# BinomialLLC/basis_universal

Hardware: AMD Instinct MI355X
Metric: encoder Mpixels/s (ETC1S frontend hot path) (higher is better)
Workload: dtype u8/int32; 1 GPU; 4096x4096 synthetic RGBA (SURVEY 8d recipe, seed 1234), ETC1S -q128 comp_level 1, basisu_frontend init+compress with tiles resident in HBM; blocks=1048576, max_endpoint_clusters=2416, max_selector_clusters=2731, final_endpoint_clusters=2413, final_selector_clusters=2277, images_in_flight_per_gpu=1, parallelism=1 x one image per GPU (no collective)

## Files before the change

basis_universal_amd/csrc/api_context.cpp:

```cpp
#include <atomic>
#include <chrono>
#include <cstdarg>
#include <cstdlib>
#include "api_internal.h"
#include "etc1s_kernels.h"
#include "tsvq_kernels.h"
#include "tsvq_bufs.h"

static std::mutex g_init_mutex;
static bool g_initialized = false;
static int g_device_count = 0;
static std::string g_global_error;
static std::atomic<int> g_live_contexts{0};
static std::mutex g_park_lock;
static std::vector<bu_hip_context*> g_parked;

void set_error(bu_hip_context* ctx, const char* fmt, ...) {
    char buf[512];
    va_list ap; va_start(ap, fmt); vsnprintf(buf, sizeof(buf), fmt, ap); va_end(ap);
    if (ctx) ctx->error = buf; else g_global_error = buf;
}

hipError_t stream_wait(bu_hip_context* ctx, hipStream_t s) {
    if (!ctx->wait_hook) return hipStreamSynchronize(s);
// ... 347 lines not shown
        ctx->tuning = default_tuning();
        std::lock_guard<std::mutex> g(g_park_lock);
        if (g_parked.size() < park_limit()) { g_parked.push_back(ctx); return; }
    }
    context_release(ctx);
}

int bu_hip_context_device(const bu_hip_context* ctx) { return ctx ? ctx->device : -1; }
int bu_hip_set_stream(bu_hip_context* ctx, void* s) {
    if (!ctx) return 0;
    (void)stream_wait(ctx, ctx->stream);
    ctx->stage_used = 0;
    ctx->stream = s ? (hipStream_t)s : ctx->own_stream;
    return 1;
}
void* bu_hip_get_stream(bu_hip_context* ctx) { return ctx ? (void*)ctx->stream : nullptr; }
const char* bu_hip_last_error(const bu_hip_context* ctx) { return ctx ? ctx->error.c_str() : g_global_error.c_str(); }
void bu_hip_set_last_error(bu_hip_context* ctx, const char* text) { set_error(ctx, "%s", text ? text : ""); }

void bu_hip_get_tuning(const bu_hip_context* ctx, bu_hip_tuning* out, uint32_t struct_bytes) {
    if (!out || struct_bytes < 8) return;
    const bu_hip_tuning& t = ctx ? ctx->tuning : default_tuning();
    std::memcpy(out, &t, std::min<size_t>(struct_bytes, sizeof(t)));
    out->struct_bytes = (uint32_t)std::min<size_t>(struct_bytes, sizeof(t));
}

int bu_hip_set_tuning(bu_hip_context* ctx, const bu_hip_tuning* t) {
    if (!ctx) return 0;
    if (!t) { ctx->tuning = default_tuning(); return 1; }
    if (t->struct_bytes < 8 || t->struct_bytes > 4096) { set_error(ctx, "bu_hip_set_tuning: struct_bytes %u", t->struct_bytes); return 0; }
    bu_hip_tuning n = default_tuning();
    std::memcpy(&n, t, std::min<size_t>(t->struct_bytes, sizeof(n)));
    n.struct_bytes = (uint32_t)sizeof(n);
    if ((n.tsvq_wide_min && n.tsvq_wide_min < 512) || (n.tsvq_wide6_min && n.tsvq_wide6_min < 512) || n.tsvq_windows > 2 || n.tsvq_poll > 2 || n.tsvq_deep_levels > bu::TSVQ_MAX_DEEP_LEVELS) {
        set_error(ctx, "bu_hip_set_tuning: value out of range (many-workgroup thresholds are 0 or >= 512, windows / poll 0..2, deep levels 0..2)");
        return 0;
    }
    ctx->tuning = n;
    return 1;
}

int bu_hip_set_wait_hook(bu_hip_context* ctx, bu_hip_wait_fn fn, void* user) {
    if (!ctx) return 0;
    ctx->wait_hook = fn; ctx->wait_user = fn ? user : nullptr;
    return 1;
}

int bu_hip_sync(bu_hip_context* ctx) {
    if (!ctx) return 0;
    device_guard g(ctx->device);
    BU_TRY(ctx, stream_wait(ctx, ctx->stream));
    return 1;
}

void* bu_hip_malloc(bu_hip_context* ctx, size_t bytes) {
    if (!ctx) return nullptr;
    device_guard g(ctx->device);
    const size_t want = ((bytes ? bytes : 1) + 255) & ~(size_t)255;
    int best = -1;
    for (size_t i = 0; i < ctx->pool_free.size(); i++) {
        const size_t cap = ctx->pool_free[i].cap;
        if (cap >= want && cap <= want * 2 + ((size_t)1 << 20) && (best < 0 || cap < ctx->pool_free[(size_t)best].cap)) best = (int)i;
    }
    if (best >= 0) {
        const bu_hip_context::pooled b = ctx->pool_free[(size_t)best];
        ctx->pool_free.erase(ctx->pool_free.begin() + best);
        ctx->pool_free_bytes -= b.cap;
        ctx->pool_live.push_back(b);
// ... 152 lines not shown
```

basis_universal_amd/csrc/api_etc1s.cpp:

```cpp
#include <atomic>
#include <cstdlib>
#include "api_internal.h"
#include "etc1s_kernels.h"
#include "mipmap_kernels.h"
#include "unique_kernels.h"
#include "bookkeeping_kernels.h"
#include "kmeans_kernels.h"
#include "host/seam_translate.h"

namespace {
constexpr uint32_t UP_PIECE_BLOCKS = 65536;
constexpr uint32_t UP_SLOTS = 8, UP_EVENTS = 64;
unsigned upload_threads() {
    static const unsigned t = [] {
        unsigned want = 4;
        if (const char* e = std::getenv("BU_UPLOAD_THREADS")) { const int v = std::atoi(e); if (v >= 1 && v <= 16) want = (unsigned)v; }
        const unsigned hw = std::thread::hardware_concurrency();
        return hw ? std::min(want, std::max(1u, hw / 2)) : 1u;
    }();
    return t;
}
bool sort_size_ok(bu_hip_context* ctx, const char* fn, uint32_t n) {
    if (n <= (1u << 30)) return true;
    set_error(ctx, "%s: %u blocks: more than 2^30 in one call", fn, n);
// ... 236 lines not shown
int bu_hip_k_refit_endpoints_given_selectors(bu_hip_context* ctx, const void* d_px, const void* d_enc, uint32_t n_clusters, const uint32_t* h_offsets,
                                             const uint32_t* d_offsets, const uint32_t* d_indices, int perceptual, uint8_t* d_params, uint64_t* d_err,
                                             uint8_t* d_valid, uint64_t* d_cur_err) {
    return bu_hip_k_refit_endpoints_given_selectors_q(ctx, d_px, d_enc, n_clusters, h_offsets, d_offsets, d_indices, BU_ETC_QUALITY_UBER, perceptual, d_params, d_err, d_valid, d_cur_err);
}

int bu_hip_k_subblock_errors(bu_hip_context* ctx, const void* d_px, uint32_t n_blocks, const uint32_t* d_block_cluster, const uint8_t* d_cluster_params,
                             int perceptual, uint64_t* d_out) {
    if (!ctx) return 0;
    device_guard g(ctx->device);
    prof_scope ps(ctx, "subblock_errors");
    BU_TRY(ctx, bu::launch_subblock_errors(ctx->stream, d_px, n_blocks, d_block_cluster, d_cluster_params, perceptual != 0, d_out));
    return 1;
}

int bu_hip_k_backend_block_errors(bu_hip_context* ctx, const void* d_px, const void* d_etc_blocks, const uint32_t* d_block_cluster, const uint8_t* d_cluster_params,
                                  uint32_t first_block, uint32_t num_blocks_x, uint32_t num_blocks_y, uint32_t n_clusters, int perceptual, int with_neighbours,
                                  uint32_t* d_own_err, uint32_t* d_neighbour_err) {
    if (!ctx) return 0;
    if (!d_px || !d_etc_blocks || !d_block_cluster || !d_cluster_params || !d_own_err || (with_neighbours && !d_neighbour_err)) { set_error(ctx, "backend_block_errors: null argument"); return 0; }
    device_guard g(ctx->device);
    prof_scope ps(ctx, "backend_block_errors");
    BU_TRY(ctx, bu::launch_backend_block_errors(ctx->stream, d_px, d_etc_blocks, d_block_cluster, d_cluster_params, first_block, num_blocks_x, num_blocks_y, n_clusters, perceptual != 0,
                                                with_neighbours != 0, d_own_err, d_neighbour_err));
    return 1;
}

int bu_hip_k_refine_endpoint_clusterization(bu_hip_context* ctx, const void* d_px, uint32_t n_blocks, const uint32_t* d_block_cluster,
                                            const uint8_t* d_cluster_params, uint32_t n_clusters, uint32_t n_parents, const uint32_t* d_cand_offsets,
                                            const uint32_t* d_cand_indices, const uint8_t* d_block_parent, int perceptual, uint32_t* d_out_best) {
    if (!ctx) return 0;
    device_guard g(ctx->device);
    void* work = nullptr;
    if (const size_t wb = ctx->tuning.refine_unsorted ? 0 : bu::refine_workspace_bytes(n_clusters, n_parents)) { BU_TRY(ctx, ctx->refine_lists.reserve(wb)); work = ctx->refine_lists.p; }
    prof_scope ps(ctx, "refine_endpoint_clusterization");
    BU_TRY(ctx, bu::launch_refine_endpoint_clusterization(ctx->stream, d_px, n_blocks, d_block_cluster, d_cluster_params, n_clusters, n_parents,
                                                          d_cand_offsets, d_cand_indices, d_block_parent, perceptual != 0, d_out_best, work));
    return 1;
}

int bu_hip_k_extract_blocks(bu_hip_context* ctx, const void* d_rgba, uint32_t width, uint32_t height, uint32_t pitch_bytes, void* d_out) {
    if (!ctx) return 0;
    if (!d_rgba || !d_out || !width || !height || pitch_bytes < width * 4u) { set_error(ctx, "extract_blocks: bad arguments"); return 0; }
    device_guard g(ctx->device);
    prof_scope ps(ctx, "extract_blocks");
    BU_TRY(ctx, bu::launch_extract_blocks(ctx->stream, d_rgba, width, height, pitch_bytes, d_out));
    return 1;
}

int bu_hip_k_extract_slices(bu_hip_context* ctx, const bu_hip_slice_source* slices, uint32_t n, void* d_out) {
    if (!ctx) return 0;
    static const char* const fn = "extract_slices";
    bu::slice_table table;
    if (!checked(ctx, [&](bu::err_text e) { return bu::build_source_slices(table, fn, slices, n, d_out, e); })) return 0;
    device_guard g(ctx->device);
    uploaded_slices d;
    if (!upload_slice_table(ctx, table, d)) return 0;
    prof_scope ps(ctx, fn);
    BU_TRY(ctx, bu::launch_extract_slices(ctx->stream, static_cast<const bu_hip_slice_source*>(d.records), d.prefix, n, table.total, d_out));
    return 1;
}

int bu_hip_k_resample_rgba8(bu_hip_context* ctx, const void* d_src, uint32_t src_w, uint32_t src_h, void* d_dst, uint32_t dst_w, uint32_t dst_h,
                            const uint32_t* x_first, const uint16_t* x_pixel, const float* x_weight, const uint32_t* y_first, const uint16_t* y_pixel, const float* y_weight,
                            int x_after_y, int srgb, const float* srgb_to_linear, const uint8_t* linear_to_srgb, uint32_t num_comps) {
    if (!ctx) return 0;
    if (!d_src || !d_dst || !src_w || !src_h || !dst_w || !dst_h || !x_first || !x_pixel || !x_weight || !y_first || !y_pixel || !y_weight || !srgb_to_linear ||
        !linear_to_srgb || num_comps < 3 || num_comps > 4 || src_w > 16384 || src_h > 16384) { set_error(ctx, "resample_rgba8: bad arguments"); return 0; }
    device_guard g(ctx->device);
    const size_t nx = x_first[dst_w], ny = y_first[dst_h];
    for (uint32_t i = 0; i < nx; i++) if (x_pixel[i] >= src_w) { set_error(ctx, "resample_rgba8: x contributor out of range"); return 0; }
// ... 310 lines not shown
    if (!ctx || !ctx->d_pixel_blocks) { if (ctx) set_error(ctx, "no pixel blocks set"); return 0; }
    device_guard g(ctx->device);
    const uint32_t n = (uint32_t)ctx->total_blocks;
    arena &in = ctx->scratch[0], &o = ctx->scratch[1];
    BU_TRY(ctx, in.reserve((size_t)n * 4));
    BU_TRY(ctx, o.reserve((size_t)n * 8));
    BU_TRY(ctx, h2d(ctx, in.p, color5_inten, (size_t)n * 4));
    BU_TRY(ctx, bu::launch_determine_selectors(ctx->stream, ctx->d_pixel_blocks, n, static_cast<const uint8_t*>(in.p), nullptr, perceptual != 0, o.p));
    if (!fetch(ctx, out, o.p, (size_t)n * 8)) return 0;
    return 1;
}

int bu_hip_refine_endpoint_clusterization(bu_hip_context* ctx, const bu_block_info* info, uint32_t total_clusters, const bu_endpoint_cluster* clusters,
                                          const uint32_t* , uint32_t* out, int perceptual) {
    if (!ctx || !ctx->d_pixel_blocks) { if (ctx) set_error(ctx, "no pixel blocks set"); return 0; }
    device_guard g(ctx->device);
    const uint32_t n = (uint32_t)ctx->total_blocks;
    if (n && !out) { set_error(ctx, "refine: null pointer"); return 0; }
    bu::seam::refine_tables t;
    if (const char* e = bu::seam::translate_refine(info, n, total_clusters, clusters, t)) { set_error(ctx, "%s", e); return 0; }
    if (!n) return 1;
    const uint32_t n_parents = t.win.n_parents();

    arena &a_par = ctx->scratch[0], &a_cur = ctx->scratch[1], &a_off = ctx->scratch[2], &a_idx = ctx->scratch[3], &a_out = ctx->scratch[4];
    arena& a_bp = ctx->scratch[5];
    BU_TRY(ctx, a_par.reserve(total_clusters * 4ull)); BU_TRY(ctx, a_cur.reserve(n * 4ull)); BU_TRY(ctx, a_off.reserve(t.win.cand_offsets.size() * 4ull));
    BU_TRY(ctx, a_idx.reserve(t.win.cand_indices.size() * 4ull + 4)); BU_TRY(ctx, a_out.reserve(n * 4ull)); BU_TRY(ctx, a_bp.reserve(n));
    BU_TRY(ctx, h2d(ctx, a_par.p, t.params.data(), total_clusters * 4ull));
    BU_TRY(ctx, h2d(ctx, a_cur.p, t.block_cur.data(), n * 4ull));
    BU_TRY(ctx, h2d(ctx, a_off.p, t.win.cand_offsets.data(), t.win.cand_offsets.size() * 4ull));
    BU_TRY(ctx, h2d(ctx, a_idx.p, t.win.cand_indices.data(), t.win.cand_indices.size() * 4ull));
    BU_TRY(ctx, h2d(ctx, a_bp.p, t.win.block_parent.data(), n));
    void* work = nullptr;
    if (const size_t wb = ctx->tuning.refine_unsorted ? 0 : bu::refine_workspace_bytes(total_clusters, n_parents)) { BU_TRY(ctx, ctx->refine_lists.reserve(wb)); work = ctx->refine_lists.p; }
    BU_TRY(ctx, bu::launch_refine_endpoint_clusterization(ctx->stream, ctx->d_pixel_blocks, n, static_cast<const uint32_t*>(a_cur.p),
                                                          static_cast<const uint8_t*>(a_par.p), total_clusters, n_parents,
                                                          static_cast<const uint32_t*>(a_off.p), static_cast<const uint32_t*>(a_idx.p),
                                                          static_cast<const uint8_t*>(a_bp.p), perceptual != 0, static_cast<uint32_t*>(a_out.p), work));
    std::vector<uint32_t> pos(n);
    if (!fetch(ctx, pos.data(), a_out.p, n * 4ull)) return 0;
    for (uint32_t b = 0; b < n; b++) out[b] = clusters[pos[b]].m_cluster_index;
    return 1;
}

int bu_hip_find_optimal_selector_clusters_for_each_block(bu_hip_context* ctx, const bu_fosc_block* info, uint32_t total_input_selectors,
                                                         const bu_fosc_selector* selectors, const uint32_t* selector_cluster_indices, uint32_t* out, int perceptual) {
    if (!ctx || !ctx->d_pixel_blocks) { if (ctx) set_error(ctx, "no pixel blocks set"); return 0; }
    device_guard g(ctx->device);
    const uint32_t n = (uint32_t)ctx->total_blocks;
    if (n && (!out || !selector_cluster_indices)) { set_error(ctx, "fosc: null pointer"); return 0; }
    bu::seam::fosc_tables t;
    if (const char* e = bu::seam::translate_fosc(info, n, total_input_selectors, selectors, t)) { set_error(ctx, "%s", e); return 0; }
    if (!n) return 1;
    const uint32_t n_parents = t.win.n_parents();

    arena &a_sel = ctx->scratch[0], &a_enc = ctx->scratch[1], &a_off = ctx->scratch[2], &a_idx = ctx->scratch[3], &a_tmp = ctx->scratch[4], &a_bp = ctx->scratch[5];
    BU_TRY(ctx, a_sel.reserve(total_input_selectors * 8ull + 8)); BU_TRY(ctx, a_enc.reserve(n * 8ull + n * 4ull)); BU_TRY(ctx, a_off.reserve(t.win.cand_offsets.size() * 4ull));
    BU_TRY(ctx, a_idx.reserve(t.win.cand_indices.size() * 4ull + 4)); BU_TRY(ctx, a_tmp.reserve(n * 4ull)); BU_TRY(ctx, a_bp.reserve(n));
    uint32_t* d_out = reinterpret_cast<uint32_t*>(static_cast<uint8_t*>(a_enc.p) + n * 8ull);
    BU_TRY(ctx, h2d(ctx, a_sel.p, t.selector_blocks.data(), total_input_selectors * 8ull));
    BU_TRY(ctx, h2d(ctx, a_enc.p, t.encoded_blocks.data(), n * 8ull));
    BU_TRY(ctx, h2d(ctx, a_off.p, t.win.cand_offsets.data(), t.win.cand_offsets.size() * 4ull));
    BU_TRY(ctx, h2d(ctx, a_idx.p, t.win.cand_indices.data(), t.win.cand_indices.size() * 4ull));
    BU_TRY(ctx, h2d(ctx, a_bp.p, t.win.block_parent.data(), n));
    BU_TRY(ctx, bu::launch_find_optimal_selector_clusters(ctx->stream, ctx->d_pixel_blocks, a_enc.p, n, a_sel.p, total_input_selectors, n_parents,
                                                          static_cast<const uint32_t*>(a_off.p), static_cast<const uint32_t*>(a_idx.p), static_cast<const uint8_t*>(a_bp.p),
                                                          perceptual != 0, 0, static_cast<uint32_t*>(a_tmp.p), d_out, nullptr, 0));
    std::vector<uint32_t> pos(n);
    if (!fetch(ctx, pos.data(), d_out, n * 4ull)) return 0;
    for (uint32_t b = 0; b < n; b++) out[b] = selector_cluster_indices[pos[b]];
    return 1;
// ... 33 lines not shown
```

basis_universal_amd/csrc/etc1s_kernels.h:

```cpp
#pragma once
#include <hip/hip_runtime.h>
#include <stdint.h>
#include <vector>
#include "../../include/basisu_hip.h"

namespace bu {

enum { BU_Q_FAST = 0, BU_Q_MEDIUM = 1, BU_Q_SLOW = 2, BU_Q_UBER = 3 };

hipError_t upload_block_fit_tables();
hipError_t upload_cluster_fit_tables();

hipError_t launch_encode_etc1s_blocks(hipStream_t st, const void* d_pixel_blocks, uint32_t n_blocks, int quality, bool perceptual, void* d_out);
hipError_t launch_endpoint_training_vectors(hipStream_t st, const void* d_etc_blocks, uint32_t n_blocks, float* d_out6);
hipError_t launch_selector_training_vectors(hipStream_t st, const void* d_enc_blocks, uint32_t n_blocks, bool perceptual, float* d_out16, uint64_t* d_w);
hipError_t launch_generate_endpoint_codebook(hipStream_t st, const void* d_pixel_blocks, uint32_t n_clusters, const uint32_t* d_order,
                                             const uint32_t* d_offsets, const uint32_t* d_indices, int quality, bool perceptual, uint32_t step,
                                             uint8_t* d_params, uint64_t* d_err, uint8_t* d_valid);
struct cb_wide_layout { size_t states_at, chunks_at, sum_at, total, image_bytes; uint32_t n_big, n_chunks; };
cb_wide_layout codebook_wide_prepare(const uint32_t* h_cluster, const uint32_t* h_first, const uint32_t* h_subblocks, uint32_t n_big, std::vector<unsigned char>& image);
hipError_t launch_codebook_wide_means(hipStream_t st, const void* d_pixel_blocks, const uint32_t* d_indices, void* d_work, const cb_wide_layout& L, float* d_out );
hipError_t launch_codebook_wide(hipStream_t st, const void* d_pixel_blocks, const uint32_t* d_indices, void* d_work, const cb_wide_layout& L, int quality, bool perceptual, bool forced,
                                uint32_t step, const void* d_enc_blocks, uint8_t* d_params, uint64_t* d_err, uint8_t* d_valid, uint64_t* d_cur_err);
hipError_t launch_refit_endpoints_given_selectors(hipStream_t st, const void* d_pixel_blocks, const void* d_enc_blocks, uint32_t n_clusters, const uint32_t* d_order,
                                                  const uint32_t* d_offsets, const uint32_t* d_indices, int quality, bool perceptual, uint8_t* d_params, uint64_t* d_err,
                                                  uint8_t* d_valid, uint64_t* d_cur_err);
hipError_t launch_subblock_errors(hipStream_t st, const void* d_pixel_blocks, uint32_t n_blocks, const uint32_t* d_block_cluster, const uint8_t* d_cluster_params,
                                  bool perceptual, uint64_t* d_out);
hipError_t launch_backend_block_errors(hipStream_t st, const void* d_pixel_blocks, const void* d_etc_blocks, const uint32_t* d_block_cluster, const uint8_t* d_cluster_params,
                                       uint32_t first_block, uint32_t nbx, uint32_t nby, uint32_t n_clusters, bool perceptual, bool with_neighbours, uint32_t* d_own,
                                       uint32_t* d_neighbour);
hipError_t launch_refine_endpoint_clusterization(hipStream_t st, const void* d_pixel_blocks, uint32_t n_blocks, const uint32_t* d_block_cluster,
                                                 const uint8_t* d_cluster_params, uint32_t n_clusters, uint32_t n_parents, const uint32_t* d_cand_offsets,
                                                 const uint32_t* d_cand_indices, const uint8_t* d_block_parent, bool perceptual, uint32_t* d_out_best,
                                                 void* d_work );
size_t refine_workspace_bytes(uint32_t n_clusters, uint32_t n_parents);
hipError_t launch_determine_selectors(hipStream_t st, const void* d_pixel_blocks, uint32_t n_blocks, const uint8_t* d_color5_inten,
                                      const uint32_t* d_block_cluster, bool perceptual, void* d_out);
size_t create_optimized_selector_codebook_workspace_bytes(uint32_t n_clusters);
hipError_t launch_create_optimized_selector_codebook(hipStream_t st, const void* d_pixel_blocks, const void* d_enc_blocks, uint32_t n_clusters,
                                                     const uint32_t* d_offsets, const uint32_t* d_block_indices, bool perceptual,
                                                     void* d_workspace, void* d_selector_blocks);
hipError_t launch_find_optimal_selector_clusters(hipStream_t st, const void* d_pixel_blocks, void* d_enc_blocks, uint32_t n_blocks,
                                                 const void* d_selector_blocks, uint32_t n_selectors, uint32_t n_parents, const uint32_t* d_cand_offsets,
                                                 const uint32_t* d_cand_indices, const uint8_t* d_block_parent, bool perceptual, uint32_t chunk,
                                                 uint32_t* d_scratch_idx, uint32_t* d_out_idx, uint32_t* d_cand_words , size_t cand_words_capacity );

hipError_t launch_extract_blocks(hipStream_t st, const void* d_rgba, uint32_t width, uint32_t height, uint32_t pitch_bytes, void* d_out_blocks);
hipError_t launch_extract_slices(hipStream_t st, const bu_hip_slice_source* d_slices, const uint32_t* d_prefix, uint32_t n_slices, uint32_t total_tiles, void* d_out_blocks);

}
```

basis_universal_amd/csrc/etc1s_refine_kernels.hip:

```cpp
#include <hip/hip_runtime.h>
#include <stdint.h>
#include "etc1s_device.h"
#include "etc1s_kernels.h"
#include "launch_dispatch.h"

namespace bu {


template <bool PERCEPTUAL>
__global__ __launch_bounds__(256) void k_refine_endpoint_clusterization(
    const uint4* __restrict__ pixel_blocks, uint32_t n_blocks, const uint32_t* __restrict__ block_cluster,
    const uint32_t* __restrict__ cluster_params, uint32_t n_clusters, uint32_t n_parents,
    const uint32_t* __restrict__ cand_offsets, const uint32_t* __restrict__ cand_indices, const uint8_t* __restrict__ block_parent,
    uint32_t* __restrict__ out_best) {
    constexpr uint32_t RQ = 256;
    __shared__ uint2 s_q[4][2][RQ];
    __shared__ uint32_t s_qp[4][2][RQ];
    const uint32_t lane = threadIdx.x & 63u;
    const uint32_t block = (uint32_t)__builtin_amdgcn_readfirstlane((int)(blockIdx.x * 4u + (threadIdx.x >> 6)));
    if (block >= n_blocks) return;

    cvec pc[16];
    {
        const uint4* src = pixel_blocks + (size_t)block * 4;
// ... 361 lines not shown
#pragma unroll
                for (int i = 0; i < 3; i++) tot += min_err4<PERCEPTUAL>(pixel_cvec<PERCEPTUAL>(block_words[(REST_PX >> (4u * (part * 3u + (uint32_t)i))) & 15u]), bc);
                tot += (uint32_t)__shfl_xor((int)tot, 1, 64);
                tot += (uint32_t)__shfl_xor((int)tot, 2, 64);
                if (have && part == 0) {
                    tot += qp[j];
                    best_key = min(best_key, ((uint64_t)tot << 32) | e.y);
                    if ((e.y & 0xffffu) == cur) cur_err = tot;
                }
            }
            if (attempt == 0) tighten();
            __builtin_amdgcn_wave_barrier();
        }
        if (seen_cur || attempt == 1) break;
        thr = 0xFFFFFFFFu; best_key = ~0ull; cur_err = 0xFFFFFFFFu;
    }
#pragma unroll
    for (int o = 32; o >= 1; o >>= 1) {
        const uint32_t lo = (uint32_t)__shfl_xor((int)(uint32_t)best_key, o, 64);
        const uint32_t hi = (uint32_t)__shfl_xor((int)(uint32_t)(best_key >> 32), o, 64);
        best_key = min(best_key, ((uint64_t)hi << 32) | lo);
        cur_err = min(cur_err, (uint32_t)__shfl_xor((int)cur_err, o, 64));
    }
    if (lane == 0) {
        const uint32_t min_err = (uint32_t)(best_key >> 32);
        uint32_t winner;
        if (best_key == ~0ull) winner = 0;
        else if (min_err != 0 && cur_err == min_err) winner = cur;
        else winner = (uint32_t)best_key & 0xffffu;
        out_best[block] = winner;
    }
}

static size_t refine_items_bytes(uint32_t n_clusters, size_t lists) { return (lists * n_clusters * sizeof(uint2) + 255) & ~(size_t)255; }

size_t refine_workspace_bytes(uint32_t n_clusters, uint32_t n_parents) {
    if (n_clusters > 65535u) return 0;
    const size_t lists = n_parents ? n_parents : 1;
    return refine_items_bytes(n_clusters, lists) + lists * RS_SEG * sizeof(uint32_t);
}

hipError_t launch_refine_endpoint_clusterization(hipStream_t st, const void* d_pixel_blocks, uint32_t n_blocks, const uint32_t* d_block_cluster,
                                                 const uint8_t* d_cluster_params, uint32_t n_clusters, uint32_t n_parents, const uint32_t* d_cand_offsets,
                                                 const uint32_t* d_cand_indices, const uint8_t* d_block_parent, bool perceptual, uint32_t* d_out_best, void* d_work) {
    if (!n_blocks) return hipSuccess;
    const dim3 grid((n_blocks + 3) / 4), blk(256);
    const uint4* in = static_cast<const uint4*>(d_pixel_blocks);
    const uint32_t* prm = reinterpret_cast<const uint32_t*>(d_cluster_params);
    const bool sorted = d_work && refine_workspace_bytes(n_clusters, n_parents);
    with_bool(perceptual, [&](auto p) {
        constexpr bool P = decltype(p)::value;
        if (sorted) {
            const size_t lists = n_parents ? n_parents : 1;
            uint2* items = static_cast<uint2*>(d_work);
            uint32_t* seg = reinterpret_cast<uint32_t*>(static_cast<char*>(d_work) + refine_items_bytes(n_clusters, lists));
            hipLaunchKernelGGL(k_refine_sort_lists<P>, dim3((uint32_t)lists), blk, 0, st, prm, n_clusters, n_parents, d_cand_offsets, d_cand_indices, items, seg);
            hipLaunchKernelGGL(k_refine_sorted<P>, grid, blk, 0, st, in, n_blocks, d_block_cluster, prm, n_parents, items, seg, d_block_parent, d_out_best);
        } else {
            hipLaunchKernelGGL(k_refine_endpoint_clusterization<P>, grid, blk, 0, st, in, n_blocks, d_block_cluster, prm, n_clusters, n_parents, d_cand_offsets, d_cand_indices,
                               d_block_parent, d_out_best);
        }
    });
    BU_LAUNCH_CHECK();
    return hipSuccess;
}

}
```

include/basisu_hip.h:

```cpp
#ifndef BASISU_HIP_H
#define BASISU_HIP_H
#include <stddef.h>
#include <stdint.h>

#ifdef __cplusplus
extern "C" {
#endif

#if defined(__GNUC__)
#define BU_HIP_API __attribute__((visibility("default")))
#else
#define BU_HIP_API
#endif


typedef struct bu_hip_context bu_hip_context;

#pragma pack(push, 1)
typedef struct { uint8_t m_pixels[16][4]; } bu_pixel_block;
typedef struct { uint8_t m_bytes[8]; } bu_etc_block;
typedef struct { uint8_t r, g, b, a; } bu_color_rgba;
typedef struct { uint64_t m_total_pixels, m_first_pixel_index; } bu_pixel_cluster;
typedef struct { uint16_t m_first_cluster_ofs, m_num_clusters, m_cur_cluster_index; uint8_t m_cur_cluster_etc_inten; } bu_block_info;
typedef struct { bu_color_rgba m_unscaled_color; uint8_t m_etc_inten; uint16_t m_cluster_index; } bu_endpoint_cluster;
// ... 100 lines not shown
    uint32_t width, height;
    uint32_t selector;
    uint32_t reserved;
} bu_hip_mip_level_record;
BU_HIP_API int bu_hip_k_prepare_mip_levels(bu_hip_context*, const void* d_payload, size_t payload_bytes, const bu_hip_mip_level_record* records, uint32_t n,
        void* d_out, size_t out_bytes, uint32_t* d_flags);

enum { BU_ETC_QUALITY_FAST = 0, BU_ETC_QUALITY_MEDIUM = 1, BU_ETC_QUALITY_SLOW = 2, BU_ETC_QUALITY_UBER = 3 };

BU_HIP_API int bu_hip_k_encode_etc1s_blocks(bu_hip_context*, const void* d_pixel_blocks, uint32_t n_blocks, int quality, int perceptual, void* d_out_etc_blocks);
BU_HIP_API int bu_hip_k_upload_and_encode_etc1s_blocks(bu_hip_context*, void* d_pixel_blocks, const void* h_pixel_blocks, uint32_t n_blocks, int quality, int perceptual,
    void* d_out_etc_blocks);
BU_HIP_API int bu_hip_k_endpoint_training_vectors(bu_hip_context*, const void* d_etc_blocks, uint32_t n_blocks, float* d_out_vec6);
BU_HIP_API int bu_hip_k_generate_endpoint_codebook(bu_hip_context*, const void* d_pixel_blocks, uint32_t n_clusters,
    const uint32_t* h_offsets, const uint32_t* d_offsets, const uint32_t* d_indices, int quality, int perceptual, uint32_t step,
    uint8_t* d_params, uint64_t* d_err, uint8_t* d_valid);
BU_HIP_API int bu_hip_k_cluster_colour_means(bu_hip_context*, const void* d_pixel_blocks, uint32_t n_clusters, const uint32_t* h_offsets, const uint32_t* d_indices, float* h_out);
BU_HIP_API int bu_hip_k_refit_endpoints_given_selectors(bu_hip_context*, const void* d_pixel_blocks, const void* d_encoded_blocks, uint32_t n_clusters,
    const uint32_t* h_offsets, const uint32_t* d_offsets, const uint32_t* d_indices, int perceptual,
    uint8_t* d_params, uint64_t* d_err, uint8_t* d_valid, uint64_t* d_current_err);
BU_HIP_API int bu_hip_k_refit_endpoints_given_selectors_q(bu_hip_context*, const void* d_pixel_blocks, const void* d_encoded_blocks, uint32_t n_clusters,
    const uint32_t* h_offsets, const uint32_t* d_offsets, const uint32_t* d_indices, int quality, int perceptual,
    uint8_t* d_params, uint64_t* d_err, uint8_t* d_valid, uint64_t* d_current_err);
BU_HIP_API int bu_hip_k_subblock_errors(bu_hip_context*, const void* d_pixel_blocks, uint32_t n_blocks, const uint32_t* d_block_cluster,
    const uint8_t* d_cluster_params, int perceptual, uint64_t* d_out_err);
BU_HIP_API int bu_hip_k_backend_block_errors(bu_hip_context*, const void* d_pixel_blocks, const void* d_etc_blocks, const uint32_t* d_block_cluster, const uint8_t* d_cluster_params,
    uint32_t first_block, uint32_t num_blocks_x, uint32_t num_blocks_y, uint32_t n_clusters, int perceptual, int with_neighbours, uint32_t* d_own_err, uint32_t* d_neighbour_err);
BU_HIP_API int bu_hip_k_generate_endpoint_codebook_part(bu_hip_context*, const void* d_pixel_blocks, uint32_t n_clusters,
    const uint32_t* h_offsets, const uint32_t* d_offsets, const uint32_t* d_indices, int quality, int perceptual, uint32_t step,
    uint8_t* d_params, uint64_t* d_err, uint8_t* d_valid, uint32_t part, uint32_t parts);
BU_HIP_API int bu_hip_k_refine_endpoint_clusterization(bu_hip_context*, const void* d_pixel_blocks, uint32_t n_blocks,
    const uint32_t* d_block_cluster, const uint8_t* d_cluster_params, uint32_t n_clusters, uint32_t n_parents,
    const uint32_t* d_cand_offsets, const uint32_t* d_cand_indices, const uint8_t* d_block_parent, int perceptual, uint32_t* d_out_best_cluster);
BU_HIP_API int bu_hip_k_resample_rgba8(bu_hip_context*, const void* d_src, uint32_t src_w, uint32_t src_h, void* d_dst, uint32_t dst_w, uint32_t dst_h,
    const uint32_t* x_first, const uint16_t* x_pixel, const float* x_weight, const uint32_t* y_first, const uint16_t* y_pixel, const float* y_weight,
    int x_after_y, int srgb, const float* srgb_to_linear_256, const uint8_t* linear_to_srgb_8192, uint32_t num_comps);
BU_HIP_API int bu_hip_k_determine_selectors(bu_hip_context*, const void* d_pixel_blocks, uint32_t n_blocks,
    const uint8_t* d_color5_inten, const uint32_t* d_block_cluster, int perceptual, void* d_out_etc_blocks);
BU_HIP_API int bu_hip_k_selector_training_vectors(bu_hip_context*, const void* d_encoded_blocks, uint32_t n_blocks, int perceptual, float* d_out_vec16, uint64_t* d_out_weight);
BU_HIP_API int bu_hip_k_create_optimized_selector_codebook(bu_hip_context*, const void* d_pixel_blocks, const void* d_encoded_blocks,
    uint32_t n_clusters, const uint32_t* d_offsets, const uint32_t* d_block_indices, int perceptual, void* d_selector_blocks);
BU_HIP_API int bu_hip_k_find_optimal_selector_clusters(bu_hip_context*, const void* d_pixel_blocks, void* d_encoded_blocks, uint32_t n_blocks,
    const void* d_selector_blocks, uint32_t n_selectors, uint32_t n_parents, const uint32_t* d_cand_offsets, const uint32_t* d_cand_indices,
    const uint8_t* d_block_parent, int perceptual, uint32_t chunk, uint32_t* d_out_block_selector_cluster);

BU_HIP_API int bu_hip_k_encode_uastc_blocks(bu_hip_context*, const void* d_pixel_blocks, uint32_t n_blocks, uint32_t flags, void* d_out_uastc_blocks);
BU_HIP_API size_t bu_hip_uastc_workspace_bytes(uint32_t n_blocks, uint32_t flags);
BU_HIP_API size_t bu_hip_uastc_rdo_workspace_bytes(uint32_t n_blocks, uint32_t total_jobs);

typedef struct bu_uastc_rdo_params {
    float m_lambda;
    float m_max_allowed_rms_increase_ratio;
    float m_skip_block_rms_thresh;
    float m_max_smooth_block_std_dev;
    float m_smooth_block_max_error_scale;
    uint32_t m_lz_dict_size;
    uint32_t m_lz_literal_cost;
    uint32_t m_endpoint_refinement;
} bu_uastc_rdo_params;
BU_HIP_API void bu_hip_uastc_rdo_default_params(bu_uastc_rdo_params* out);
BU_HIP_API int bu_hip_k_uastc_rdo(bu_hip_context*, void* d_uastc_blocks, const void* d_pixel_blocks, uint32_t n_blocks, const bu_uastc_rdo_params* params,
                                  uint32_t flags, uint32_t total_jobs, uint32_t out_stats[4]);
BU_HIP_API int bu_hip_k_uastc_rdo_slices(bu_hip_context*, void* d_uastc_blocks, const void* d_pixel_blocks, const uint32_t* slice_blocks, uint32_t n_slices,
                                         const bu_uastc_rdo_params* params, uint32_t flags, uint32_t total_jobs, uint32_t* out_stats);
BU_HIP_API size_t bu_hip_uastc_rdo_slices_workspace_bytes(const uint32_t* slice_blocks, uint32_t n_slices, uint32_t total_jobs);
BU_HIP_API int bu_hip_uastc_rdo(bu_hip_context*, bu_uastc_block* blocks, const bu_uastc_rdo_params* params, uint32_t flags, uint32_t total_jobs,
// ... 213 lines not shown
```

Before: 1240 Mpixels/s.

## Bucket blocks by parent and table for lane-per-block refine with candidate queues

Adds a new default refine path for perceptual mode. Blocks are counting-sorted into buckets keyed by parent and the current cluster's intensity table. A new kernel then gives each wave lane one block, scans the bucket's sorted candidate list uniformly across the wave, and queues candidates that pass a chroma lower bound (or a partial clamped error) in shared memory before evaluating the full error. This is meant to cut divergence and redundant full-error evaluations compared with the previous sorted kernel. In exchange it adds extra sort kernels, a memset and more workspace, and runs a second pass over the lists when a block's current cluster is not in its candidate list.

```diff
diff --git a/basis_universal_amd/csrc/api_context.cpp b/basis_universal_amd/csrc/api_context.cpp
--- a/basis_universal_amd/csrc/api_context.cpp
+++ b/basis_universal_amd/csrc/api_context.cpp
@@ -403,8 +403,8 @@
     bu_hip_tuning n = default_tuning();
     std::memcpy(&n, t, std::min<size_t>(t->struct_bytes, sizeof(n)));
     n.struct_bytes = (uint32_t)sizeof(n);
-    if ((n.tsvq_wide_min && n.tsvq_wide_min < 512) || (n.tsvq_wide6_min && n.tsvq_wide6_min < 512) || n.tsvq_windows > 2 || n.tsvq_poll > 2 || n.tsvq_deep_levels > bu::TSVQ_MAX_DEEP_LEVELS) {
-        set_error(ctx, "bu_hip_set_tuning: value out of range (many-workgroup thresholds are 0 or >= 512, windows / poll 0..2, deep levels 0..2)");
+    if ((n.tsvq_wide_min && n.tsvq_wide_min < 512) || (n.tsvq_wide6_min && n.tsvq_wide6_min < 512) || n.tsvq_windows > 2 || n.tsvq_poll > 2 || n.refine_unsorted > 2 || n.tsvq_deep_levels > bu::TSVQ_MAX_DEEP_LEVELS) {
+        set_error(ctx, "bu_hip_set_tuning: value out of range (many-workgroup thresholds are 0 or >= 512, windows / poll / refine_unsorted 0..2, deep levels 0..2)");
         return 0;
     }
     ctx->tuning = n;
diff --git a/basis_universal_amd/csrc/api_etc1s.cpp b/basis_universal_amd/csrc/api_etc1s.cpp
--- a/basis_universal_amd/csrc/api_etc1s.cpp
+++ b/basis_universal_amd/csrc/api_etc1s.cpp
@@ -292,11 +292,18 @@
     if (!ctx) return 0;
     device_guard g(ctx->device);
     void* work = nullptr;
-    if (const size_t wb = ctx->tuning.refine_unsorted ? 0 : bu::refine_workspace_bytes(n_clusters, n_parents)) { BU_TRY(ctx, ctx->refine_lists.reserve(wb)); work = ctx->refine_lists.p; }
+    const int path = bu_hip_refine_path(ctx, n_clusters, n_parents, perceptual);
+    if (path != 1) { BU_TRY(ctx, ctx->refine_lists.reserve(bu::refine_workspace_bytes(n_clusters, n_parents, n_blocks))); work = ctx->refine_lists.p; }
     prof_scope ps(ctx, "refine_endpoint_clusterization");
     BU_TRY(ctx, bu::launch_refine_endpoint_clusterization(ctx->stream, d_px, n_blocks, d_block_cluster, d_cluster_params, n_clusters, n_parents,
-                                                          d_cand_offsets, d_cand_indices, d_block_parent, perceptual != 0, d_out_best, work));
-    return 1;
+                                                          d_cand_offsets, d_cand_indices, d_block_parent, perceptual != 0, d_out_best, path, work));
+    return 1;
+}
+
+int bu_hip_refine_path(const bu_hip_context* ctx, uint32_t n_clusters, uint32_t n_parents, int perceptual) {
+    bu_hip_tuning t;
+    bu_hip_get_tuning(ctx, &t, sizeof(t));
+    return bu::refine_path(t.refine_unsorted, n_clusters, n_parents, perceptual != 0);
 }
 
 int bu_hip_k_extract_blocks(bu_hip_context* ctx, const void* d_rgba, uint32_t width, uint32_t height, uint32_t pitch_bytes, void* d_out) {
@@ -673,11 +680,12 @@
     BU_TRY(ctx, h2d(ctx, a_idx.p, t.win.cand_indices.data(), t.win.cand_indices.size() * 4ull));
     BU_TRY(ctx, h2d(ctx, a_bp.p, t.win.block_parent.data(), n));
     void* work = nullptr;
-    if (const size_t wb = ctx->tuning.refine_unsorted ? 0 : bu::refine_workspace_bytes(total_clusters, n_parents)) { BU_TRY(ctx, ctx->refine_lists.reserve(wb)); work = ctx->refine_lists.p; }
+    const int path = bu_hip_refine_path(ctx, total_clusters, n_parents, perceptual);
+    if (path != 1) { BU_TRY(ctx, ctx->refine_lists.reserve(bu::refine_workspace_bytes(total_clusters, n_parents, n))); work = ctx->refine_lists.p; }
     BU_TRY(ctx, bu::launch_refine_endpoint_clusterization(ctx->stream, ctx->d_pixel_blocks, n, static_cast<const uint32_t*>(a_cur.p),
                                                           static_cast<const uint8_t*>(a_par.p), total_clusters, n_parents,
                                                           static_cast<const uint32_t*>(a_off.p), static_cast<const uint32_t*>(a_idx.p),
-                                                          static_cast<const uint8_t*>(a_bp.p), perceptual != 0, static_cast<uint32_t*>(a_out.p), work));
+                                                          static_cast<const uint8_t*>(a_bp.p), perceptual != 0, static_cast<uint32_t*>(a_out.p), path, work));
     std::vector<uint32_t> pos(n);
     if (!fetch(ctx, pos.data(), a_out.p, n * 4ull)) return 0;
     for (uint32_t b = 0; b < n; b++) out[b] = clusters[pos[b]].m_cluster_index;
diff --git a/basis_universal_amd/csrc/etc1s_kernels.h b/basis_universal_amd/csrc/etc1s_kernels.h
--- a/basis_universal_amd/csrc/etc1s_kernels.h
+++ b/basis_universal_amd/csrc/etc1s_kernels.h
@@ -33,8 +33,9 @@
 hipError_t launch_refine_endpoint_clusterization(hipStream_t st, const void* d_pixel_blocks, uint32_t n_blocks, const uint32_t* d_block_cluster,
                                                  const uint8_t* d_cluster_params, uint32_t n_clusters, uint32_t n_parents, const uint32_t* d_cand_offsets,
                                                  const uint32_t* d_cand_indices, const uint8_t* d_block_parent, bool perceptual, uint32_t* d_out_best,
-                                                 void* d_work );
-size_t refine_workspace_bytes(uint32_t n_clusters, uint32_t n_parents);
+                                                 int path , void* d_work );
+int refine_path(uint32_t refine_unsorted, uint32_t n_clusters, uint32_t n_parents, bool perceptual);
+size_t refine_workspace_bytes(uint32_t n_clusters, uint32_t n_parents, uint32_t n_blocks);
 hipError_t launch_determine_selectors(hipStream_t st, const void* d_pixel_blocks, uint32_t n_blocks, const uint8_t* d_color5_inten,
                                       const uint32_t* d_block_cluster, bool perceptual, void* d_out);
 size_t create_optimized_selector_codebook_workspace_bytes(uint32_t n_clusters);
diff --git a/basis_universal_amd/csrc/etc1s_refine_kernels.hip b/basis_universal_amd/csrc/etc1s_refine_kernels.hip
--- a/basis_universal_amd/csrc/etc1s_refine_kernels.hip
+++ b/basis_universal_amd/csrc/etc1s_refine_kernels.hip
@@ -417,28 +417,324 @@
     }
 }
 
+
+constexpr uint32_t RB_MAX_BUCKETS = 2048;
+constexpr uint32_t RB_TILE = 1024;
+constexpr uint32_t RB_QCAP = 12;
+
+__device__ __forceinline__ uint32_t refine_bucket_key(uint32_t b, const uint32_t* __restrict__ block_cluster, const uint32_t* __restrict__ cluster_params, uint32_t n_parents,
+                                                      const uint8_t* __restrict__ block_parent) {
+    const uint32_t parent = n_parents ? min((uint32_t)block_parent[b], n_parents - 1u) : 0u;
+    return parent * 8u + ((cluster_params[block_cluster[b]] >> 24) & 7u);
+}
+
+__global__ __launch_bounds__(256) void k_refine_bucket_count(uint32_t n_blocks, const uint32_t* __restrict__ block_cluster, const uint32_t* __restrict__ cluster_params,
+                                                             uint32_t n_parents, const uint8_t* __restrict__ block_parent, uint32_t n_buckets, uint16_t* __restrict__ keys,
+                                                             uint32_t* __restrict__ counts) {
+    __shared__ uint32_t s_cnt[RB_MAX_BUCKETS];
+    const uint32_t tid = threadIdx.x;
+    for (uint32_t i = tid; i < n_buckets; i += 256) s_cnt[i] = 0;
+    __syncthreads();
+    for (uint32_t i = 0; i < RB_TILE / 256; i++) {
+        const uint32_t b = blockIdx.x * RB_TILE + i * 256u + tid;
+        if (b < n_blocks) {
+            const uint32_t key = refine_bucket_key(b, block_cluster, cluster_params, n_parents, block_parent);
+            keys[b] = (uint16_t)key;
+            atomicAdd(&s_cnt[key], 1u);
+        }
+    }
+    __syncthreads();
+    for (uint32_t i = tid; i < n_buckets; i += 256) if (s_cnt[i]) atomicAdd(&counts[i], s_cnt[i]);
+}
+
+__global__ __launch_bounds__(256) void k_refine_bucket_scan(const uint32_t* __restrict__ counts, uint32_t n_buckets, uint32_t* __restrict__ bstart, uint32_t* __restrict__ wstart,
+                                                            uint32_t* __restrict__ cursor) {
+    __shared__ uint32_t s_b[256], s_w[256];
+    const uint32_t tid = threadIdx.x, k0 = tid * (RB_MAX_BUCKETS / 256);
+    uint32_t sb = 0, sw = 0;
+    for (uint32_t k = k0; k < min(k0 + RB_MAX_BUCKETS / 256, n_buckets); k++) { const uint32_t c = counts[k]; sb += c; sw += (c + 63u) >> 6; }
+    s_b[tid] = sb; s_w[tid] = sw;
+    __syncthreads();
+    for (uint32_t o = 1; o < 256; o <<= 1) {
+        const uint32_t vb = tid >= o ? s_b[tid - o] : 0u, vw = tid >= o ? s_w[tid - o] : 0u;
+        __syncthreads();
+        s_b[tid] += vb; s_w[tid] += vw;
+        __syncthreads();
+    }
+    uint32_t rb = s_b[tid] - sb, rw = s_w[tid] - sw;
+    for (uint32_t k = k0; k < min(k0 + RB_MAX_BUCKETS / 256, n_buckets); k++) {
+        const uint32_t c = counts[k];
+        bstart[k] = rb; cursor[k] = rb; wstart[k] = rw;
+        rb += c; rw += (c + 63u) >> 6;
+    }
+    if (tid == 255) { bstart[n_buckets] = s_b[255]; wstart[n_buckets] = s_w[255]; }
+}
+
+__global__ __launch_bounds__(256) void k_refine_bucket_scatter(uint32_t n_blocks, const uint16_t* __restrict__ keys, uint32_t n_buckets, uint32_t* __restrict__ cursor,
+                                                               uint32_t* __restrict__ ids) {
+    __shared__ uint32_t s_cnt[RB_MAX_BUCKETS];
+    const uint32_t tid = threadIdx.x;
+    for (uint32_t i = tid; i < n_buckets; i += 256) s_cnt[i] = 0;
+    __syncthreads();
+    uint32_t key[RB_TILE / 256], rank[RB_TILE / 256];
+#pragma unroll
+    for (uint32_t i = 0; i < RB_TILE / 256; i++) {
+        const uint32_t b = blockIdx.x * RB_TILE + i * 256u + tid;
+        key[i] = 0; rank[i] = 0;
+        if (b < n_blocks) { key[i] = min((uint32_t)keys[b], n_buckets - 1u); rank[i] = atomicAdd(&s_cnt[key[i]], 1u); }
+    }
+    __syncthreads();
+    for (uint32_t i = tid; i < n_buckets; i += 256) { const uint32_t c = s_cnt[i]; if (c) s_cnt[i] = atomicAdd(&cursor[i], c); }
+    __syncthreads();
+#pragma unroll
+    for (uint32_t i = 0; i < RB_TILE / 256; i++) {
+        const uint32_t b = blockIdx.x * RB_TILE + i * 256u + tid;
+        if (b < n_blocks) ids[s_cnt[key[i]] + rank[i]] = b;
+    }
+}
+
+__device__ __forceinline__ int inten_a64(uint32_t table) { return (int)((uint32_t)(0x2F2118120D090502ull >> (table * 8u)) & 255u) << 6; }
+__device__ __forceinline__ int inten_b64(uint32_t table) { return (int)((uint32_t)(0xB76A503C2A1D1108ull >> (table * 8u)) & 255u) << 6; }
+__device__ __forceinline__ cvec entry_base_cvec(uint32_t prm) {
+    return to_cvec<true>(scale5((int)(prm & 255u)), scale5((int)((prm >> 8) & 255u)), scale5((int)((prm >> 16) & 255u)));
+}
+__device__ __forceinline__ int mul24_lane(int a, int b) {
+    asm("" : "+v"(a));
+    asm("" : "+v"(b));
+    return __mul24(a, b);
+}
+__device__ __forceinline__ uint32_t sq24_lane(int a) {
+    asm("" : "+v"(a));
+    return (uint32_t)__mul24(a, a);
+}
+__device__ __forceinline__ uint32_t lane_chroma_term(int dy, int dz) {
+    const uint32_t cr = sq24_lane(dy) >> 5, cb = sq24_lane(dz) >> 5;
+    uint32_t cr5 = (cr << 2) + cr;
+    asm("" : "+v"(cr5));
+    return (((cr << 4) + (cr5 << 1)) >> 7) + (((cb << 1) + cb) >> 7);
+}
+__device__ __forceinline__ uint32_t lane_cdist(const cvec& a, const cvec& b) {
+    return (sq24_lane(a.x - b.x) >> 5) + lane_chroma_term(a.y - b.y, a.z - b.z);
+}
+__device__ __forceinline__ uint32_t lane_min_err4(const cvec& p, const cvec bc[4]) {
+    return min(min(lane_cdist(p, bc[0]), lane_cdist(p, bc[1])), min(lane_cdist(p, bc[2]), lane_cdist(p, bc[3])));
+}
+__device__ __forceinline__ uint32_t unclamped_term(const cvec& p, const cvec& bcv, int a64, int b64) {
+    const int dx0 = p.x - bcv.x, m = dx0 < 0 ? -dx0 : dx0;
+    return (min(sq24_lane(m - a64), sq24_lane(m - b64)) >> 5) + lane_chroma_term(p.y - bcv.y, p.z - bcv.z);
+}
+__device__ __forceinline__ uint32_t lane_chroma_lower_bound(const chroma_moments& t, int cy, int cz) {
+    const int ey = t.my - cy, ez = t.mz - cz;
+    const int A = (int)(sq24_lane(ey) >> 6) + t.r2y + (mul24_lane(ey, t.r1y) >> 9);
+    const int B = (int)(sq24_lane(ez) >> 6) + t.r2z + (mul24_lane(ez, t.r1z) >> 9);
+    return (uint32_t)max(((__mul24(A, 26) + __mul24(B, 3)) >> 2) - 36, 0);
+}
+__device__ __forceinline__ void entry_clamped_cvecs(cvec out[4], uint32_t prm) {
+    const uint32_t table = (prm >> 24) & 7u;
+    const int a = inten_a64(table) >> 6, b = inten_b64(table) >> 6;
+    const int br = scale5((int)(prm & 255u)), bg = scale5((int)((prm >> 8) & 255u)), bb = scale5((int)((prm >> 16) & 255u));
+    out[0] = to_cvec<true>(clamp255(br - b), clamp255(bg - b), clamp255(bb - b));
+    out[1] = to_cvec<true>(clamp255(br - a), clamp255(bg - a), clamp255(bb - a));
+    out[2] = to_cvec<true>(clamp255(br + a), clamp255(bg + a), clamp255(bb + a));
+    out[3] = to_cvec<true>(clamp255(br + b), clamp255(bg + b), clamp255(bb + b));
+}
+
+__global__ __launch_bounds__(256) void k_refine_block_lanes(const uint4* __restrict__ pixel_blocks, const uint32_t* __restrict__ block_cluster,
+                                                            const uint32_t* __restrict__ cluster_params, const uint2* __restrict__ items, const uint32_t* __restrict__ seg,
+                                                            const uint32_t* __restrict__ ids, const uint32_t* __restrict__ bstart, const uint32_t* __restrict__ wstart,
+                                                            uint32_t n_buckets, uint32_t* __restrict__ out_best) {
+    __shared__ uint32_t s_qj[4][RB_QCAP * 64];
+    __shared__ uint32_t s_qb[4][RB_QCAP * 64];
+    const uint32_t lane = threadIdx.x & 63u;
+    const uint32_t wave = (uint32_t)__builtin_amdgcn_readfirstlane((int)(blockIdx.x * 4u + (threadIdx.x >> 6)));
+    if (wave >= wstart[n_buckets]) return;
+    uint32_t bucket;
+    {
+        uint32_t lo = 0, hi = n_buckets;
+        while (hi - lo > 1u) {
+            const uint32_t mid = (lo + hi) >> 1;
+            if (wstart[mid] <= wave) lo = mid; else hi = mid;
+        }
+        bucket = (uint32_t)__builtin_amdgcn_readfirstlane((int)lo);
+    }
+    const uint32_t table = bucket & 7u;
+    const uint32_t* sg = seg + (size_t)(bucket >> 3) * RS_SEG;
+    const uint32_t first = sg[0], plain_total = sg[1], n_plain = sg[2 + table], n_clamped = sg[10 + table];
+    const uint2* plain_items = items + first;
+    const uint2* clamped_items = items + first + plain_total;
+    const uint32_t b0 = bstart[bucket], at = (wave - wstart[bucket]) * 64u + lane;
+    const bool valid = at < bstart[bucket + 1] - b0;
+    const uint32_t block = ids[b0 + (valid ? at : 0u)];
+
+    cvec pc[16];
+    {
+        const uint4* src = pixel_blocks + (size_t)block * 4;
+#pragma unroll
+        for (int i = 0; i < 4; i++) {
+            const uint4 v = src[i];
+            pc[i * 4 + 0] = pixel_cvec<true>(v.x); pc[i * 4 + 1] = pixel_cvec<true>(v.y);
+            pc[i * 4 + 2] = pixel_cvec<true>(v.z); pc[i * 4 + 3] = pixel_cvec<true>(v.w);
+        }
+    }
+    chroma_moments cm = { 0, 0, 0, 0, 0, 0 };
+    {
+        int s1y = 0, s1z = 0;
+#pragma unroll
+        for (int i = 0; i < 16; i++) { s1y += pc[i].y; s1z += pc[i].z; }
+        cm.my = s1y >> 4; cm.mz = s1z >> 4; cm.r1y = s1y - 16 * cm.my; cm.r1z = s1z - 16 * cm.mz;
+#pragma unroll
+        for (int i = 0; i < 16; i++) {
+            const int ry = pc[i].y - cm.my, rz = pc[i].z - cm.mz;
+            cm.r2y += (int)(sq24_lane(ry) >> 10); cm.r2z += (int)(sq24_lane(rz) >> 10);
+        }
+    }
+    const uint32_t cur = block_cluster[block];
+    auto plain_error = [&](uint32_t prm) {
+        const uint32_t t = (prm >> 24) & 7u;
+        const cvec bcv = entry_base_cvec(prm);
+        const int a64 = inten_a64(t), b64 = inten_b64(t);
+        uint32_t tot = 0;
+#pragma unroll
+        for (int i = 0; i < 16; i++) tot += unclamped_term(pc[i], bcv, a64, b64);
+        return tot;
+    };
+    uint32_t thr;
+    {
+        const uint32_t cur_prm = cluster_params[cur];
+        const int b = inten_b64(table) >> 6;
+        const int cr = scale5((int)(cur_prm & 255u)), cg = scale5((int)((cur_prm >> 8) & 255u)), cb = scale5((int)((cur_prm >> 16) & 255u));
+        if (min(cr, min(cg, cb)) - b >= 0 && max(cr, max(cg, cb)) + b <= 255) {
+            thr = plain_error(cur_prm);
+        } else {
+            cvec bc[4];
+            entry_clamped_cvecs(bc, cur_prm);
+            thr = 0;
+#pragma unroll
+            for (int i = 0; i < 16; i++) thr += lane_min_err4(pc[i], bc);
+        }
+    }
+    uint32_t* qj = s_qj[threadIdx.x >> 6] + lane;
+    uint32_t* qb = s_qb[threadIdx.x >> 6] + lane;
+    uint64_t best_key = ~0ull;
+    uint32_t cur_err = 0xFFFFFFFFu;
+    uint32_t cnt = 0;
+    bool live = valid, seen_cur = false;
+    auto take = [&](uint32_t tot, uint32_t y) {
+        best_key = min(best_key, ((uint64_t)tot << 32) | y);
+        if ((y & 0xffffu) == cur) cur_err = tot;
+        thr = min(thr, tot);
+    };
+#pragma unroll 1
+    for (int attempt = 0; attempt < 2; attempt++) {
+        uint2 next = n_plain ? plain_items[0] : make_uint2(0u, 0u);
+#pragma unroll 1
+        for (uint32_t j = 0; j <= n_plain; j++) {
+            if (j < n_plain) {
+                const uint2 e = next;
+                next = plain_items[min(j + 1u, n_plain - 1u)];
+                const cvec bcv = entry_base_cvec(e.x);
+                const uint32_t bound = lane_chroma_lower_bound(cm, bcv.y, bcv.z);
+                seen_cur = seen_cur || (e.y & 0xffffu) == cur;
+                if (live && bound <= thr) { qj[cnt * 64u] = j; qb[cnt * 64u] = bound; cnt++; }
+            }
+            if (j == n_plain || __ballot(cnt == RB_QCAP) != 0ull) {
+                for (uint32_t s = 0; __ballot(s < cnt) != 0ull; s++) {
+                    if (s < cnt && qb[s * 64u] <= thr) {
+                        const uint2 e = plain_items[qj[s * 64u]];
+                        take(plain_error(e.x), e.y);
+                    }
+                }
+                cnt = 0;
+            }
+        }
+        next = n_clamped ? clamped_items[0] : make_uint2(0u, 0u);
+#pragma unroll 1
+        for (uint32_t j = 0; j <= n_clamped; j++) {
+            if (j < n_clamped) {
+                const uint2 e = next;
+                next = clamped_items[min(j + 1u, n_clamped - 1u)];
+                cvec bc[4];
+                entry_clamped_cvecs(bc, e.x);
+                uint32_t part = 0;
+#pragma unroll
+                for (int f = 0; f < 4; f++) part += lane_min_err4(pc[f * 5], bc);
+                seen_cur = seen_cur || (e.y & 0xffffu) == cur;
+                if (live && part <= thr) { qj[cnt * 64u] = j; qb[cnt * 64u] = part; cnt++; }
+            }
+            if (j == n_clamped || __ballot(cnt == RB_QCAP) != 0ull) {
+                for (uint32_t s = 0; __ballot(s < cnt) != 0ull; s++) {
+                    if (s < cnt && qb[s * 64u] <= thr) {
+                        const uint2 e = clamped_items[qj[s * 64u]];
+                        cvec bc[4];
+                        entry_clamped_cvecs(bc, e.x);
+                        uint32_t tot = qb[s * 64u];
+#pragma unroll
+                        for (int i = 0; i < 16; i++) if (i % 5) tot += lane_min_err4(pc[i], bc);
+                        take(tot, e.y);
+                    }
+                }
+                cnt = 0;
+            }
+        }
+        live = valid && !seen_cur;
+        if (attempt == 1 || __ballot(live) == 0ull) break;
+        if (live) { thr = 0xFFFFFFFFu; best_key = ~0ull; cur_err = 0xFFFFFFFFu; }
+    }
+    if (valid) {
+        const uint32_t min_err = (uint32_t)(best_key >> 32);
+        uint32_t winner;
+        if (best_key == ~0ull) winner = 0;
+        else if (min_err != 0 && cur_err == min_err) winner = cur;
+        else winner = (uint32_t)best_key & 0xffffu;
+        out_best[block] = winner;
+    }
+}
+
 static size_t refine_items_bytes(uint32_t n_clusters, size_t lists) { return (lists * n_clusters * sizeof(uint2) + 255) & ~(size_t)255; }
-
-size_t refine_workspace_bytes(uint32_t n_clusters, uint32_t n_parents) {
+static size_t refine_lists_bytes(uint32_t n_clusters, size_t lists) { return (refine_items_bytes(n_clusters, lists) + lists * RS_SEG * sizeof(uint32_t) + 255) & ~(size_t)255; }
+constexpr size_t RB_TABLES_BYTES = (2 * RB_MAX_BUCKETS + 2 * (RB_MAX_BUCKETS + 64)) * sizeof(uint32_t);
+
+int refine_path(uint32_t refine_unsorted, uint32_t n_clusters, uint32_t n_parents, bool perceptual) {
+    if (refine_unsorted == 1 || n_clusters > 65535u) return 1;
+    return refine_unsorted == 2 || !perceptual || n_parents * 8u > RB_MAX_BUCKETS ? 2 : 0;
+}
+
+size_t refine_workspace_bytes(uint32_t n_clusters, uint32_t n_parents, uint32_t n_blocks) {
     if (n_clusters > 65535u) return 0;
     const size_t lists = n_parents ? n_parents : 1;
-    return refine_items_bytes(n_clusters, lists) + lists * RS_SEG * sizeof(uint32_t);
+    return refine_lists_bytes(n_clusters, lists) + RB_TABLES_BYTES + (size_t)n_blocks * (sizeof(uint32_t) + sizeof(uint16_t));
 }
 
 hipError_t launch_refine_endpoint_clusterization(hipStream_t st, const void* d_pixel_blocks, uint32_t n_blocks, const uint32_t* d_block_cluster,
                                                  const uint8_t* d_cluster_params, uint32_t n_clusters, uint32_t n_parents, const uint32_t* d_cand_offsets,
-                                                 const uint32_t* d_cand_indices, const uint8_t* d_block_parent, bool perceptual, uint32_t* d_out_best, void* d_work) {
+                                                 const uint32_t* d_cand_indices, const uint8_t* d_block_parent, bool perceptual, uint32_t* d_out_best, int path, void* d_work) {
     if (!n_blocks) return hipSuccess;
+    if (path != refine_path((uint32_t)path, n_clusters, n_parents, perceptual) || (path != 1 && !d_work)) return hipErrorInvalidValue;
     const dim3 grid((n_blocks + 3) / 4), blk(256);
     const uint4* in = static_cast<const uint4*>(d_pixel_blocks);
     const uint32_t* prm = reinterpret_cast<const uint32_t*>(d_cluster_params);
-    const bool sorted = d_work && refine_workspace_bytes(n_clusters, n_parents);
+    const size_t lists = n_parents ? n_parents : 1;
+    uint2* items = static_cast<uint2*>(d_work);
+    uint32_t* seg = reinterpret_cast<uint32_t*>(static_cast<char*>(d_work) + refine_items_bytes(n_clusters, lists));
+    if (path == 0) {
+        const uint32_t n_buckets = (uint32_t)lists * 8u;
+        uint32_t* counts = reinterpret_cast<uint32_t*>(static_cast<char*>(d_work) + refine_lists_bytes(n_clusters, lists));
+        uint32_t *cursor = counts + RB_MAX_BUCKETS, *bstart = cursor + RB_MAX_BUCKETS, *wstart = bstart + RB_MAX_BUCKETS + 64, *ids = wstart + RB_MAX_BUCKETS + 64;
+        uint16_t* keys = reinterpret_cast<uint16_t*>(ids + n_blocks);
+        const dim3 tiles((n_blocks + RB_TILE - 1) / RB_TILE);
+        const uint32_t waves = (n_blocks + 63u) / 64u + n_buckets;
+        if (hipError_t e = hipMemsetAsync(counts, 0, n_buckets * sizeof(uint32_t), st)) return e;
+        hipLaunchKernelGGL(k_refine_sort_lists<true>, dim3((uint32_t)lists), blk, 0, st, prm, n_clusters, n_parents, d_cand_offsets, d_cand_indices, items, seg);
+        hipLaunchKernelGGL(k_refine_bucket_count, tiles, blk, 0, st, n_blocks, d_block_cluster, prm, n_parents, d_block_parent, n_buckets, keys, counts);
+        hipLaunchKernelGGL(k_refine_bucket_scan, dim3(1), blk, 0, st, counts, n_buckets, bstart, wstart, cursor);
+        hipLaunchKernelGGL(k_refine_bucket_scatter, tiles, blk, 0, st, n_blocks, keys, n_buckets, cursor, ids);
+        hipLaunchKernelGGL(k_refine_block_lanes, dim3((waves + 3) / 4), blk, 0, st, in, d_block_cluster, prm, items, seg, ids, bstart, wstart, n_buckets, d_out_best);
+        BU_LAUNCH_CHECK();
+        return hipSuccess;
+    }
     with_bool(perceptual, [&](auto p) {
         constexpr bool P = decltype(p)::value;
-        if (sorted) {
-            const size_t lists = n_parents ? n_parents : 1;
-            uint2* items = static_cast<uint2*>(d_work);
-            uint32_t* seg = reinterpret_cast<uint32_t*>(static_cast<char*>(d_work) + refine_items_bytes(n_clusters, lists));
+        if (path == 2) {
             hipLaunchKernelGGL(k_refine_sort_lists<P>, dim3((uint32_t)lists), blk, 0, st, prm, n_clusters, n_parents, d_cand_offsets, d_cand_indices, items, seg);
             hipLaunchKernelGGL(k_refine_sorted<P>, grid, blk, 0, st, in, n_blocks, d_block_cluster, prm, n_parents, items, seg, d_block_parent, d_out_best);
         } else {
diff --git a/include/basisu_hip.h b/include/basisu_hip.h
--- a/include/basisu_hip.h
+++ b/include/basisu_hip.h
@@ -156,6 +156,7 @@
 BU_HIP_API int bu_hip_k_refine_endpoint_clusterization(bu_hip_context*, const void* d_pixel_blocks, uint32_t n_blocks,
     const uint32_t* d_block_cluster, const uint8_t* d_cluster_params, uint32_t n_clusters, uint32_t n_parents,
     const uint32_t* d_cand_offsets, const uint32_t* d_cand_indices, const uint8_t* d_block_parent, int perceptual, uint32_t* d_out_best_cluster);
+BU_HIP_API int bu_hip_refine_path(const bu_hip_context*, uint32_t n_clusters, uint32_t n_parents, int perceptual);
 BU_HIP_API int bu_hip_k_resample_rgba8(bu_hip_context*, const void* d_src, uint32_t src_w, uint32_t src_h, void* d_dst, uint32_t dst_w, uint32_t dst_h,
     const uint32_t* x_first, const uint16_t* x_pixel, const float* x_weight, const uint32_t* y_first, const uint16_t* y_pixel, const float* y_weight,
     int x_after_y, int srgb, const float* srgb_to_linear_256, const uint8_t* linear_to_srgb_8192, uint32_t num_comps);
```

New measurement: 1322 Mpixels/s, median of 6. 1.07x the previous value.
